# Lainshower/debiasing-multi-modal

Hardware: AMD Instinct MI355X
Metric: images/sec (embed+adapter step), CLIP-RN50 224px bs=1024 (higher is better)
Workload: dtype f32; 1 GPU; CLIP-RN50 224px encode_image + adapter(1024-128-1024) CE/SGD step, 1024 images/GPU, global batch 1024 (the metric's configuration, CLIP-RN50 224px bs=1024 on one GPU); global_batch=1024, batch_per_gpu=1024, parallelism=dp1, collective=none

## Files before the change

### debiasing-multi-modal_amd/csrc/bottleneck_chain.hip

```cpp
#include <stdlib.h>
#include "common.h"

namespace {

struct ChainP {
    const float* a; const float* a_absmax;
    const u16* w3; int w3_exp; const float* sc3; const float* b3;
    const float* res; float* x; float* xp; float* x_absmax;
    const u16* w1; int w1_exp; const float* sc1; const float* b1;
    float* y1; float* y1_absmax;
    int M, N;
    int Ho, Wo;
    const float* a2; const float* a2_absmax; const u16* wd; const float* ratio;
    const u16* w2; int w2_exp; const float* sc2; const float* b2;
    int H, W;
};

template <int RH>
__device__ __forceinline__ int swz(int row) { return RH == 32 ? ((row >> 2) & 3) : (RH == 64 ? ((row >> 1) & 7) : (row & 15)); }

constexpr int BM = 128;

template <int K, int P>
struct ChainGeo {
    static constexpr int BNS = K == 64 ? 64 : 32;
    static constexpr int SLROW = BNS + 4;
    static constexpr int R1_BYTES = BM * SLROW * 4 > 2 * BM * 64 * 2 ? BM * SLROW * 4 : 2 * BM * 64 * 2;
    static constexpr int W3_BYTES = BNS * K * 2;
    static constexpr int W1_BYTES = P * BNS * 2;
    static constexpr int LDS_BYTES = R1_BYTES + W3_BYTES + W1_BYTES;
};

template <int POOL>
__device__ __forceinline__ int row_pixel(const ChainP& p, int m) {
    if constexpr (!POOL) return m;
    const int mp = m >> 2, q = m & 3, wp2 = p.Wo >> 1, hwp = (p.Ho >> 1) * wp2;
    const int n = mp / hwp, rem = mp - n * hwp, hp = rem / wp2;
    return (n * p.Ho + 2 * hp + (q >> 1)) * p.Wo + 2 * (rem - hp * wp2) + (q & 1);
}

constexpr int C2_SROWS = 132, C2_PLANE = C2_SROWS * 32;
constexpr int C2_W2P = 104;
template <int K>
struct Conv2Geo {
    static constexpr int W2_OFF = 2 * C2_PLANE;
    static constexpr int GROUP_BYTES = (2 * C2_PLANE * 2 + K * C2_W2P * 2 + 255) / 256 * 256;
    static constexpr int NST = K == 64 ? 2 : 1;
    static constexpr int Z_OFF = NST * GROUP_BYTES;
    static constexpr int BYTES = Z_OFF + 256;
    static constexpr int STAGE_BYTES = BM * 68 * 4;
};
constexpr int cmax(int a, int b) { return a > b ? a : b; }

template <int K, int P, int POOL, int DUAL = 0, int CONV2 = 0>
__global__ __launch_bounds__(256, 2) void bottleneck_chain_kernel(const ChainP p) {
    static_assert(!DUAL || K == 64, "dual-source variant: layer-1 geometry (K = K2 = 64)");
    static_assert(!CONV2 || !POOL, "the conv2 phase walks pixels in standard order");
    static_assert(K == 64 || K == 128, "conv3 reduction depth: 64 (layer 1) or 128 (layer 2)");
    static_assert(P == 64 || P == 128, "conv1' width");
    using G = ChainGeo<K, P>;
    constexpr int BNS = G::BNS, SLROW = G::SLROW;
    constexpr int KS = K / 16, TN3 = BNS / 32, TN1 = P / 32;
    constexpr int LDS_TOTAL = cmax(G::LDS_BYTES + (DUAL ? BNS * 64 * 2 : 0), CONV2 ? cmax(Conv2Geo<K>::BYTES, Conv2Geo<K>::STAGE_BYTES) : 0);
    __shared__ __attribute__((aligned(256))) unsigned char lds_raw[LDS_TOTAL];
    u16* Ay = (u16*)lds_raw;
    float* slab = (float*)lds_raw;
    u16* W3b = (u16*)(lds_raw + G::R1_BYTES);
    u16* W1b = (u16*)(lds_raw + G::R1_BYTES + G::W3_BYTES);
    u16* Wdb = (u16*)(lds_raw + G::R1_BYTES + G::W3_BYTES + G::W1_BYTES);

    const int tid = threadIdx.x, lane = tid & 63, wave = tid >> 6;
    const int fr = lane & 31, fh = lane >> 5;
    const int m0 = xcd_remap(blockIdx.x, gridDim.x) * BM;
    const int NT = p.N / BNS;

    const int g0 = row_pixel<POOL>(p, m0);
    const long long Mll = p.M;
    const __amdgpu_buffer_rsrc_t rsA = desc(p.a, Mll * K * 4, (long long)g0 * K * 4);
    const __amdgpu_buffer_rsrc_t rsR = DUAL ? desc(p.a2, Mll * 64 * 4, (long long)g0 * 64 * 4)
                                            : desc(p.res, Mll * p.N * 4, (long long)g0 * p.N * 4);
    const __amdgpu_buffer_rsrc_t rsX = desc(p.x, POOL == 2 ? 0 : Mll * p.N * 4, (long long)g0 * p.N * 4);
    const __amdgpu_buffer_rsrc_t rsY = desc(p.y1, Mll * P * 4, (long long)g0 * P * 4);
    __amdgpu_buffer_rsrc_t rsXP = rsX;
    if constexpr (POOL) rsXP = desc(p.xp, (Mll >> 2) * p.N * 4, (long long)(m0 >> 2) * p.N * 4);

    unsigned gx[4], gy[4];
#pragma unroll
    for (int t = 0; t < 4; ++t) {
        const int m = m0 + wave * 32 + 8 * t + 4 * fh;
        const int dp = row_pixel<POOL>(p, m) - g0;
        gx[t] = m < p.M ? (unsigned)dp * (unsigned)(p.N * 4) + (unsigned)(fr * 4) : OOR;
        gy[t] = m < p.M ? (unsigned)dp * (unsigned)(P * 4) + (unsigned)(fr * 4) : OOR;
    }
    auto qpix = [&](int q) { return POOL ? (q >> 1) * p.Wo + (q & 1) : q; };

    constexpr int CPR3 = K / 8, RPP3 = 256 / CPR3, W3LD = BNS * CPR3 / 256;
    constexpr int CPR1 = BNS / 8, RPP1 = 256 / CPR1, W1LD = P * CPR1 / 256;
    static_assert(W3LD >= 1 && W1LD >= 1, "weight slabs smaller than one pass of the workgroup");
    const int wc3 = tid % CPR3, wr3 = tid / CPR3, wc1 = tid % CPR1, wr1 = tid / CPR1;
    u32x4 w3r[W3LD], w1r[W1LD], wdr[DUAL ? W3LD : 1];
    auto load_w = [&](int nt) {
#pragma unroll
        for (int j = 0; j < W3LD; ++j) {
            w3r[j] = *(const u32x4*)(p.w3 + (size_t)(nt * BNS + wr3 + RPP3 * j) * K + wc3 * 8);
            if constexpr (DUAL) wdr[j] = *(const u32x4*)(p.wd + (size_t)(nt * BNS + wr3 + RPP3 * j) * 64 + wc3 * 8);
        }
#pragma unroll
        for (int j = 0; j < W1LD; ++j)
            w1r[j] = *(const u32x4*)(p.w1 + (size_t)(wr1 + RPP1 * j) * p.N + nt * BNS + wc1 * 8);
    };
    auto store_w = [&]() {
#pragma unroll
        for (int j = 0; j < W3LD; ++j) {
            const int row = wr3 + RPP3 * j;
            *(u32x4*)(W3b + row * K + ((wc3 ^ swz<K>(row)) << 3)) = w3r[j];
            if constexpr (DUAL) *(u32x4*)(Wdb + row * 64 + ((wc3 ^ swz<64>(row)) << 3)) = wdr[j];
        }
#pragma unroll
        for (int j = 0; j < W1LD; ++j) {
            const int row = wr1 + RPP1 * j;
            *(u32x4*)(W1b + row * BNS + ((wc1 ^ swz<BNS>(row)) << 3)) = w1r[j];
        }
    };
    load_w(0);
    float rr[DUAL ? 1 : TN3][16];
    auto load_res = [&](int nt) {
        if constexpr (DUAL) return;
#pragma unroll
        for (int j = 0; j < TN3; ++j)
#pragma unroll
            for (int r = 0; r < 16; ++r)
                rr[j][r] = __builtin_bit_cast(float, __builtin_amdgcn_raw_buffer_load_b32(
                    rsR, gx[r >> 2], (unsigned)((nt * BNS + j * 32) * 4 + qpix(r & 3) * p.N * 4), 0));
    };
    load_res(0);
    u32x4 af[KS][2], af2[DUAL ? 4 : 1][2];
    bool first_pass = true;
    auto stage_issue = [&](const __amdgpu_buffer_rsrc_t& rs, int ldk, int k0, f32x4 (&q)[8]) {
        const int lc = tid & 15, lr = tid >> 4;
#pragma unroll
        for (int i = 0; i < 8; ++i) {
            const int row = lr + 16 * i, m = m0 + row;
            const unsigned off = m < p.M ? (unsigned)(row_pixel<POOL>(p, m) - g0) * (unsigned)(ldk * 4) + lc * 16u : OOR;
            q[i] = __builtin_bit_cast(f32x4, __builtin_amdgcn_raw_buffer_load_b128(rs, off, (unsigned)(k0 * 4), 0));
        }
    };
    auto stage_finish = [&](const f32x4 (&q)[8], float sc, u32x4 (*dst)[2]) {
        const int lc = tid & 15, lr = tid >> 4;
        if (!first_pass) __syncthreads();
#pragma unroll
        for (int i = 0; i < 8; ++i) {
            const int row = lr + 16 * i;
            unsigned hp[2], lp[2];
#pragma unroll
            for (int j = 0; j < 2; ++j) split2h_pair(q[i][2 * j], q[i][2 * j + 1], sc, hp[j], lp[j]);
            const int off = row * 64 + (((lc >> 1) ^ swz<64>(row)) << 3) + ((lc & 1) << 2);
            *(u32x2*)(Ay + off) = (u32x2){hp[0], hp[1]};
            *(u32x2*)(Ay + BM * 64 + off) = (u32x2){lp[0], lp[1]};
        }
        if (first_pass) store_w();
        first_pass = false;
        __syncthreads();
#pragma unroll
        for (int ks = 0; ks < 4; ++ks) {
            const int row = wave * 32 + fr;
            const int off = row * 64 + (((2 * ks + fh) ^ swz<64>(row)) << 3);
            dst[ks][0] = *(const u32x4*)(Ay + off);
            dst[ks][1] = *(const u32x4*)(Ay + BM * 64 + off);
        }
    };
    auto stage_pass = [&](const __amdgpu_buffer_rsrc_t& rs, int ldk, int k0, float sc, u32x4 (*dst)[2]) {
        f32x4 q[8];
        stage_issue(rs, ldk, k0, q);
        stage_finish(q, sc, dst);
    };
    f32x4 q2[(DUAL && CONV2) ? 8 : 1];
    if constexpr (DUAL && CONV2) stage_issue(rsR, 64, 0, q2);
    int s_a;
    if constexpr (!CONV2) {
        s_a = scale_exp(*p.a_absmax);
#pragma unroll
        for (int kp = 0; kp < K / 64; ++kp) stage_pass(rsA, K, kp * 64, pow2f(s_a), af + kp * 4);
    } else {
        using C2 = Conv2Geo<K>;
        constexpr int TN2 = K / 32, NG = (K / 32) * 3, W2LD = (K * 12 + 255) / 256;
        u16* Sp = (u16*)lds_raw;
        constexpr int NST = C2::NST, STH = C2::GROUP_BYTES / 2;
        constexpr int ZLH = C2::Z_OFF / 2;
        if (tid < 16) *(u32x4*)(lds_raw + C2::Z_OFF + tid * 16) = (u32x4){0u, 0u, 0u, 0u};
        const int s_y1 = scale_exp(*p.a_absmax);
        const float y1_sc = pow2f(s_y1);
        const int px0 = m0 - 1 - p.W > 0 ? m0 - 1 - p.W : 0;
        const __amdgpu_buffer_rsrc_t rsS = desc(p.a, Mll * K * 4, (long long)px0 * K * 4);
        const int lc = tid & 7, lr = tid >> 3;
        unsigned s_off[5];
#pragma unroll
        for (int i = 0; i < 5; ++i) {
            const int j = lr + 32 * i;
            s_off[i] = j < 130 ? (unsigned)((m0 - 1 + j - px0) * (K * 4)) + lc * 16u : OOR;
        }
        unsigned fmask = 0;
        {
            const int m = m0 + wave * 32 + fr;
            if (m < p.M) {
                const int hw = p.H * p.W, rem = m - (m / hw) * hw, ho = rem / p.W, wo = rem - ho * p.W;
#pragma unroll
                for (int kh = 0; kh < 3; ++kh)
#pragma unroll
                    for (int kw = 0; kw < 3; ++kw)
                        if (ho + kh - 1 >= 0 && ho + kh - 1 < p.H && wo + kw - 1 >= 0 && wo + kw - 1 < p.W) fmask |= 1u << (kh * 3 + kw);
            }
        }
        f32x4 sq[5];
        u32x4 w2q[W2LD];
        auto load_group = [&](int g) {
            const int sl = g / 3, kh = g - sl * 3;
            const unsigned delta = (unsigned)(((kh - 1) * p.W * K + sl * 32) * 4);
#pragma unroll
            for (int i = 0; i < 5; ++i)
                sq[i] = __builtin_bit_cast(f32x4, __builtin_amdgcn_raw_buffer_load_b128(rsS, s_off[i] == OOR ? OOR : s_off[i] + delta, 0, 0));
#pragma unroll
            for (int i = 0; i < W2LD; ++i) {
                const int idx = tid + 256 * i, row = idx / 12, c = idx - row * 12;
                w2q[i] = idx < K * 12 ? *(const u32x4*)(p.w2 + (size_t)row * (9 * K) + (size_t)g * 96 + c * 8) : (u32x4){0u, 0u, 0u, 0u};
            }
        };
        auto store_group = [&](int st) {
            u16* Sps = Sp + st * STH;
            u16* W2b = Sps + C2::W2_OFF;
#pragma unroll
            for (int i = 0; i < 5; ++i) {
                const int row = lr + 32 * i;
                if (row < 130) {
                    unsigned hp[2], lp[2];
#pragma unroll
                    for (int j = 0; j < 2; ++j) split2h_pair(sq[i][2 * j], sq[i][2 * j + 1], y1_sc, hp[j], lp[j]);
                    const int off = row * 32 + (((lc >> 1) ^ swz<32>(row)) << 3) + ((lc & 1) << 2);
                    *(u32x2*)(Sps + off) = (u32x2){hp[0], hp[1]};
                    *(u32x2*)(Sps + C2_PLANE + off) = (u32x2){lp[0], lp[1]};
                }
            }
#pragma unroll
            for (int i = 0; i < W2LD; ++i) {
                const int idx = tid + 256 * i, row = idx / 12, c = idx - row * 12;
                if (idx < K * 12) *(u32x4*)(W2b + row * C2_W2P + c * 8) = w2q[i];
            }
        };
        f32x16 acc2[TN2];
#pragma unroll
        for (int j = 0; j < TN2; ++j)
#pragma unroll
            for (int r = 0; r < 16; ++r) acc2[j][r] = 0.f;
        auto compute_group = [&](int g, int st) {
            const u16* Sps = Sp + st * STH;
            const u16* W2b = Sps + C2::W2_OFF;
            const int zl = ZLH - st * STH;
            const int kh = g % 3;
#pragma unroll
            for (int kw = 0; kw < 3; ++kw) {
                const bool ok = (fmask >> (kh * 3 + kw)) & 1u;
                const int row = wave * 32 + fr + kw;
#pragma unroll
                for (int ks = 0; ks < 2; ++ks) {
                    const int addr = row * 32 + (((2 * ks + fh) ^ swz<32>(row)) << 3);
                    const int a0 = ok ? addr : zl + (addr & 127), a1 = ok ? addr + C2_PLANE : zl + (addr & 127);
                    const u32x4 ah = *(const u32x4*)(Sps + a0), al = *(const u32x4*)(Sps + a1);
                    u32x4 wf[TN2];
#pragma unroll
                    for (int j = 0; j < TN2; ++j) wf[j] = *(const u32x4*)(W2b + (j * 32 + fr) * C2_W2P + kw * 32 + (2 * ks + fh) * 8);
#pragma unroll
                    for (int j = 0; j < TN2; ++j)
                        acc2[j] = __builtin_amdgcn_mfma_f32_32x32x16_f16(__builtin_bit_cast(f16x8, al), __builtin_bit_cast(f16x8, wf[j]), acc2[j], 0, 0, 0);
#pragma unroll
                    for (int j = 0; j < TN2; ++j)
                        acc2[j] = __builtin_amdgcn_mfma_f32_32x32x16_f16(__builtin_bit_cast(f16x8, ah), __builtin_bit_cast(f16x8, wf[j]), acc2[j], 0, 0, 0);
                }
            }
        };
        load_group(0);
        if constexpr (NST == 2) {
            store_group(0);
            __syncthreads();
            for (int g = 0; g < NG; ++g) {
                if (g + 1 < NG) load_group(g + 1);
                compute_group(g, g & 1);
                if (g + 1 < NG) store_group((g + 1) & 1);
                __syncthreads();
            }
        } else {
            for (int g = 0; g < NG; ++g) {
                store_group(0);
                __syncthreads();
                if (g + 1 < NG) load_group(g + 1);
                compute_group(g, 0);
                __syncthreads();
            }
        }
        const float c2_scale = pow2f(-s_y1 - p.w2_exp);
        float ymax = 0.f;
#pragma unroll
        for (int j = 0; j < TN2; ++j) {
            const float sv = p.sc2[j * 32 + fr] * c2_scale, bv = p.b2[j * 32 + fr];
#pragma unroll
            for (int r = 0; r < 16; ++r) {
                float v = fmaxf(fmaf(acc2[j][r], sv, bv), 0.f);
                if (gx[r >> 2] == OOR) v = 0.f;
                acc2[j][r] = v;
                ymax = fmaxf(ymax, v);
            }
        }
        s_a = scale_exp(wave_max(ymax));
        const float y2_sc = pow2f(s_a);
        float* St = (float*)lds_raw + wave * (32 * 68);
#pragma unroll
        for (int h = 0; h < K / 64; ++h) {
#pragma unroll
            for (int jj = 0; jj < 2; ++jj)
#pragma unroll
                for (int r = 0; r < 16; ++r) St[((r & 3) + 8 * (r >> 2) + 4 * fh) * 68 + jj * 32 + fr] = acc2[2 * h + jj][r];
#pragma unroll
            for (int ks = 0; ks < 4; ++ks) {
                const f32x4 x0 = *(const f32x4*)(St + fr * 68 + 16 * ks + 8 * fh), x1 = *(const f32x4*)(St + fr * 68 + 16 * ks + 8 * fh + 4);
                unsigned hh[4], ll[4];
                split2h_pair(x0[0], x0[1], y2_sc, hh[0], ll[0]); split2h_pair(x0[2], x0[3], y2_sc, hh[1], ll[1]);
                split2h_pair(x1[0], x1[1], y2_sc, hh[2], ll[2]); split2h_pair(x1[2], x1[3], y2_sc, hh[3], ll[3]);
                af[4 * h + ks][0] = (u32x4){hh[0], hh[1], hh[2], hh[3]};
                af[4 * h + ks][1] = (u32x4){ll[0], ll[1], ll[2], ll[3]};
            }
        }
        __syncthreads();
        if constexpr (!DUAL) store_w();
    }
    float dual_dyn = 1.f;
    if constexpr (DUAL) {
        const int s_a2 = scale_exp(*p.a2_absmax);
        if constexpr (CONV2) stage_finish(q2, pow2f(s_a2), af2);
        else stage_pass(rsR, 64, 0, pow2f(s_a2), af2);
        dual_dyn = pow2f(s_a - s_a2);
    }
    __syncthreads();

    float* Ls = slab + wave * (32 * SLROW);
    const float acc3_scale = pow2f(-s_a - p.w3_exp);
    f32x16 acc1[TN1];
#pragma unroll
    for (int j = 0; j < TN1; ++j)
#pragma unroll
        for (int r = 0; r < 16; ++r) acc1[j][r] = 0.f;
    float run_max = 0.f, x_amax = 0.f;
    int s_cur = 0;

    for (int nt = 0; nt < NT; ++nt) {
        const int n0 = nt * BNS;
        if (nt + 1 < NT) load_w(nt + 1);
        f32x16 acc3[TN3];
#pragma unroll
        for (int j = 0; j < TN3; ++j)
#pragma unroll
            for (int r = 0; r < 16; ++r) acc3[j][r] = 0.f;
        if constexpr (DUAL) {
#pragma unroll
            for (int ks = 0; ks < 4; ++ks) {
                u32x4 wf[TN3];
#pragma unroll
                for (int j = 0; j < TN3; ++j) {
                    const int row = j * 32 + fr;
                    wf[j] = *(const u32x4*)(Wdb + row * 64 + (((2 * ks + fh) ^ swz<64>(row)) << 3));
                }
#pragma unroll
                for (int pl = 1; pl >= 0; --pl)
#pragma unroll
                    for (int j = 0; j < TN3; ++j)
                        acc3[j] = __builtin_amdgcn_mfma_f32_32x32x16_f16(__builtin_bit_cast(f16x8, af2[ks][pl]),
                                                                         __builtin_bit_cast(f16x8, wf[j]), acc3[j], 0, 0, 0);
            }
#pragma unroll
            for (int j = 0; j < TN3; ++j) {
                const float rt = p.ratio[n0 + j * 32 + fr] * dual_dyn;
#pragma unroll
                for (int r = 0; r < 16; ++r) acc3[j][r] *= rt;
            }
        }
#pragma unroll
        for (int ks = 0; ks < KS; ++ks) {
            u32x4 wf[TN3];
#pragma unroll
            for (int j = 0; j < TN3; ++j) {
                const int row = j * 32 + fr;
                wf[j] = *(const u32x4*)(W3b + row * K + (((2 * ks + fh) ^ swz<K>(row)) << 3));
            }
#pragma unroll
            for (int pl = 1; pl >= 0; --pl)
#pragma unroll
                for (int j = 0; j < TN3; ++j)
                    acc3[j] = __builtin_amdgcn_mfma_f32_32x32x16_f16(__builtin_bit_cast(f16x8, af[ks][pl]),
                                                                     __builtin_bit_cast(f16x8, wf[j]), acc3[j], 0, 0, 0);
        }
        float tmax = 0.f;
#pragma unroll
        for (int j = 0; j < TN3; ++j) {
            const int n = n0 + j * 32 + fr;
            const float sv = p.sc3[n] * acc3_scale, bv = p.b3[n];
#pragma unroll
            for (int r = 0; r < 16; ++r) {
                float v = fmaxf(fmaf(acc3[j][r], sv, bv) + (DUAL ? 0.f : rr[j][r]), 0.f);
                if (gx[r >> 2] == OOR) v = 0.f;
                acc3[j][r] = v;
                tmax = fmaxf(tmax, v);
                if constexpr (POOL != 2)
                    __builtin_amdgcn_raw_buffer_store_b32(__builtin_bit_cast(unsigned, v), rsX, gx[r >> 2],
                                                          (unsigned)((n0 + j * 32) * 4 + qpix(r & 3) * p.N * 4), 0);
                Ls[((r & 3) + 8 * (r >> 2) + 4 * fh) * SLROW + j * 32 + fr] = v;
            }
            if constexpr (POOL) {
#pragma unroll
                for (int t = 0; t < 4; ++t) {
                    const float s = (((acc3[j][4 * t] + acc3[j][4 * t + 1]) + acc3[j][4 * t + 2]) + acc3[j][4 * t + 3]) * 0.25f;
                    const int mp = wave * 8 + 2 * t + fh;
                    const unsigned off = gx[t] != OOR ? (unsigned)mp * (unsigned)(p.N * 4) + (unsigned)(fr * 4) : OOR;
                    __builtin_amdgcn_raw_buffer_store_b32(__builtin_bit_cast(unsigned, s), rsXP, off, (unsigned)((n0 + j * 32) * 4), 0);
                }
            }
        }
        if (nt + 1 < NT) load_res(nt + 1);
        tmax = wave_max(tmax);
        x_amax = fmaxf(x_amax, tmax);
        if (tmax > run_max) {
            run_max = tmax;
            const int s_new = scale_exp(run_max);
            if (s_new != s_cur) {
                const float f = pow2f(s_new - s_cur);
#pragma unroll
                for (int j = 0; j < TN1; ++j)
#pragma unroll
                    for (int r = 0; r < 16; ++r) acc1[j][r] *= f;
                s_cur = s_new;
            }
        }
        const float t_sc = pow2f(s_cur);
#pragma unroll
        for (int ks = 0; ks < BNS / 16; ++ks) {
            const f32x4 x0 = *(const f32x4*)(Ls + fr * SLROW + 16 * ks + 8 * fh);
            const f32x4 x1 = *(const f32x4*)(Ls + fr * SLROW + 16 * ks + 8 * fh + 4);
            unsigned h[4], l[4];
            split2h_pair(x0[0], x0[1], t_sc, h[0], l[0]); split2h_pair(x0[2], x0[3], t_sc, h[1], l[1]);
            split2h_pair(x1[0], x1[1], t_sc, h[2], l[2]); split2h_pair(x1[2], x1[3], t_sc, h[3], l[3]);
            const u32x4 ah = {h[0], h[1], h[2], h[3]}, al = {l[0], l[1], l[2], l[3]};
            u32x4 wf[TN1];
#pragma unroll
            for (int j = 0; j < TN1; ++j) {
                const int row = j * 32 + fr;
                wf[j] = *(const u32x4*)(W1b + row * BNS + (((2 * ks + fh) ^ swz<BNS>(row)) << 3));
            }
#pragma unroll
            for (int j = 0; j < TN1; ++j)
                acc1[j] = __builtin_amdgcn_mfma_f32_32x32x16_f16(__builtin_bit_cast(f16x8, al), __builtin_bit_cast(f16x8, wf[j]),
                                                                 acc1[j], 0, 0, 0);
#pragma unroll
            for (int j = 0; j < TN1; ++j)
                acc1[j] = __builtin_amdgcn_mfma_f32_32x32x16_f16(__builtin_bit_cast(f16x8, ah), __builtin_bit_cast(f16x8, wf[j]),
                                                                 acc1[j], 0, 0, 0);
        }
        __syncthreads();
        if (nt + 1 < NT) store_w();
        __syncthreads();
    }

    float y_amax = 0.f;
    const float acc1_scale = pow2f(-s_cur - p.w1_exp);
#pragma unroll
    for (int j = 0; j < TN1; ++j) {
        const int n = j * 32 + fr;
        const float sv = p.sc1[n] * acc1_scale, bv = p.b1[n];
#pragma unroll
        for (int r = 0; r < 16; ++r) {
            const float v = fmaxf(fmaf(acc1[j][r], sv, bv), 0.f);
            __builtin_amdgcn_raw_buffer_store_b32(__builtin_bit_cast(unsigned, v), rsY, gy[r >> 2],
                                                  (unsigned)(j * 32 * 4 + qpix(r & 3) * P * 4), 0);
            if (gy[r >> 2] != OOR) y_amax = fmaxf(y_amax, v);
        }
    }
    y_amax = wave_max(y_amax);
    float* red = (float*)W3b;
    if (lane == 0) { red[wave] = x_amax; red[4 + wave] = y_amax; }
    __syncthreads();
    if (tid == 0) {
        const float xm = fmaxf(fmaxf(red[0], red[1]), fmaxf(red[2], red[3]));
        const float ym = fmaxf(fmaxf(red[4], red[5]), fmaxf(red[6], red[7]));
        if (p.x_absmax && xm > *(volatile const float*)p.x_absmax) atomicMax((unsigned*)p.x_absmax, __float_as_uint(xm));
        if (p.y1_absmax && ym > *(volatile const float*)p.y1_absmax) atomicMax((unsigned*)p.y1_absmax, __float_as_uint(ym));
    }
}

}

int dbmm_chain8_launch(const float* y2, const float* y2_absmax, const void* w3_plane_f16, int w3_exp, const float* scale3,
                       const float* bias3, const float* residual, float* x_out, float* x_absmax, const void* w1_plane_f16, int w1_exp,
                       const float* scale1, const float* bias1, float* y1_out, float* y1_absmax, int64_t M, int64_t N, void* stream);

extern "C" int dbmm_bottleneck_block_chain_x2(const float* y1, const float* y1_absmax, const void* w2_plane_f16, int w2_exp,
                                              const float* scale2, const float* bias2, const void* w3_plane_f16, int w3_exp,
                                              const float* scale3, const float* bias3, const float* residual, const float* a2,
                                              const float* a2_absmax, const void* wd_plane_f16, const float* ratio, float* x_out,
                                              float* x_absmax, const void* w1_plane_f16, int w1_exp, const float* scale1,
                                              const float* bias1, float* y1_out, float* y1_out_absmax, int64_t B, int64_t H,
                                              int64_t W, int64_t K, int64_t N, int64_t P, void* stream) {
    const bool dual = a2 != nullptr;
    if (!y1 || !y1_absmax || !w2_plane_f16 || !scale2 || !bias2 || !w3_plane_f16 || !scale3 || !bias3 || !x_out || !w1_plane_f16 ||
        !scale1 || !bias1 || !y1_out)
        return DBMM_E_ARG;
    if (dual ? (!a2_absmax || !wd_plane_f16 || !ratio || residual) : (!residual || a2_absmax || wd_plane_f16 || ratio)) return DBMM_E_ARG;
    if (B <= 0 || H <= 0 || W <= 0 || K <= 0 || N <= 0 || P <= 0) return DBMM_E_SHAPE;
    const int64_t M = B * H * W;
    if (M > (INT32_MAX >> 1)) return DBMM_E_SHAPE;
    const bool served = dual ? (K == 64 && P == 64) : ((K == 64 && P == 64) || (K == 128 && P == 128));
    if (!served || (N % 64) != 0 || (M & 3)) return DBMM_E_UNSUPPORTED;
    if (w2_exp < -40 || w2_exp > 40 || w3_exp < -40 || w3_exp > 40 || w1_exp < -40 || w1_exp > 40) return DBMM_E_UNSUPPORTED;
    if (!dbmm_aligned16(y1) || !dbmm_aligned16(w2_plane_f16) || !dbmm_aligned16(w3_plane_f16) || !dbmm_aligned16(w1_plane_f16) ||
        !dbmm_aligned16(x_out) || !dbmm_aligned16(y1_out) || (residual && !dbmm_aligned16(residual)) || (a2 && !dbmm_aligned16(a2)) ||
        (wd_plane_f16 && !dbmm_aligned16(wd_plane_f16)))
        return DBMM_E_ALIGN;
    ChainP p{};
    p.a = y1; p.a_absmax = y1_absmax;
    p.w2 = (const u16*)w2_plane_f16; p.w2_exp = w2_exp; p.sc2 = scale2; p.b2 = bias2; p.H = (int)H; p.W = (int)W;
    p.w3 = (const u16*)w3_plane_f16; p.w3_exp = w3_exp; p.sc3 = scale3; p.b3 = bias3;
    p.res = residual; p.a2 = a2; p.a2_absmax = a2_absmax; p.wd = (const u16*)wd_plane_f16; p.ratio = ratio;
    p.x = x_out; p.x_absmax = x_absmax;
    p.w1 = (const u16*)w1_plane_f16; p.w1_exp = w1_exp; p.sc1 = scale1; p.b1 = bias1;
    p.y1 = y1_out; p.y1_absmax = y1_out_absmax;
    p.M = (int)M; p.N = (int)N; p.Ho = (int)H; p.Wo = (int)W;
    const dim3 grid((unsigned)((M + BM - 1) / BM));
    hipStream_t s = (hipStream_t)stream;
    if (dual) hipLaunchKernelGGL((bottleneck_chain_kernel<64, 64, 0, 1, 1>), grid, dim3(256), 0, s, p);
    else if (K == 64) hipLaunchKernelGGL((bottleneck_chain_kernel<64, 64, 0, 0, 1>), grid, dim3(256), 0, s, p);
    else hipLaunchKernelGGL((bottleneck_chain_kernel<128, 128, 0, 0, 1>), grid, dim3(256), 0, s, p);
    DBMM_CHECK_LAUNCH();
    return DBMM_OK;
}

extern "C" int dbmm_bottleneck_chain_dual_x2(const float* y2, const float* y2_absmax, const void* w3_plane_f16, int w3_exp,
                                             const float* scale3, const float* bias, const float* a2, const float* a2_absmax,
                                             const void* wd_plane_f16, const float* ratio, float* x_out, float* x_absmax,
                                             const void* w1_plane_f16, int w1_exp, const float* scale1, const float* bias1,
                                             float* y1_out, float* y1_absmax, int64_t M, int64_t K, int64_t K2, int64_t N,
                                             int64_t P, void* stream) {
    if (!y2 || !y2_absmax || !w3_plane_f16 || !scale3 || !bias || !a2 || !a2_absmax || !wd_plane_f16 || !ratio || !x_out ||
        !w1_plane_f16 || !scale1 || !bias1 || !y1_out)
        return DBMM_E_ARG;
    if (M <= 0 || K <= 0 || K2 <= 0 || N <= 0 || P <= 0 || M > (INT32_MAX >> 1)) return DBMM_E_SHAPE;
    if (K != 64 || K2 != 64 || (N % 64) != 0 || (P != 64 && P != 128) || (M & 3)) return DBMM_E_UNSUPPORTED;
    if (w3_exp < -40 || w3_exp > 40 || w1_exp < -40 || w1_exp > 40) return DBMM_E_UNSUPPORTED;
    if (!dbmm_aligned16(y2) || !dbmm_aligned16(a2) || !dbmm_aligned16(w3_plane_f16) || !dbmm_aligned16(wd_plane_f16) ||
        !dbmm_aligned16(w1_plane_f16) || !dbmm_aligned16(x_out) || !dbmm_aligned16(y1_out))
        return DBMM_E_ALIGN;
    ChainP p{};
    p.a = y2; p.a_absmax = y2_absmax;
    p.w3 = (const u16*)w3_plane_f16; p.w3_exp = w3_exp; p.sc3 = scale3; p.b3 = bias;
    p.a2 = a2; p.a2_absmax = a2_absmax; p.wd = (const u16*)wd_plane_f16; p.ratio = ratio;
    p.x = x_out; p.x_absmax = x_absmax;
    p.w1 = (const u16*)w1_plane_f16; p.w1_exp = w1_exp; p.sc1 = scale1; p.b1 = bias1;
    p.y1 = y1_out; p.y1_absmax = y1_absmax;
    p.M = (int)M; p.N = (int)N; p.Ho = 1; p.Wo = (int)M;
    const dim3 grid((unsigned)((M + BM - 1) / BM));
    hipStream_t s = (hipStream_t)stream;
    if (P == 64) hipLaunchKernelGGL((bottleneck_chain_kernel<64, 64, 0, 1>), grid, dim3(256), 0, s, p);
    else hipLaunchKernelGGL((bottleneck_chain_kernel<64, 128, 0, 1>), grid, dim3(256), 0, s, p);
    DBMM_CHECK_LAUNCH();
    return DBMM_OK;
}

extern "C" int dbmm_bottleneck_chain_x2(const float* y2, const float* y2_absmax, const void* w3_plane_f16, int w3_exp,
                                        const float* scale3, const float* bias3, const float* residual, float* x_out,
                                        float* x_pooled, float* x_absmax, const void* w1_plane_f16, int w1_exp,
                                        const float* scale1, const float* bias1, float* y1_out, float* y1_absmax,
                                        int64_t B, int64_t Ho, int64_t Wo, int64_t K, int64_t N, int64_t P, void* stream) {
    if (!y2 || !y2_absmax || !w3_plane_f16 || !scale3 || !bias3 || !residual || !w1_plane_f16 || !scale1 || !bias1 || !y1_out)
        return DBMM_E_ARG;
    if (!x_out && !x_pooled) return DBMM_E_ARG;
    if (B <= 0 || Ho <= 0 || Wo <= 0 || K <= 0 || N <= 0 || P <= 0) return DBMM_E_SHAPE;
    const int64_t M = B * Ho * Wo;
    if (M > (INT32_MAX >> 1)) return DBMM_E_SHAPE;
    if (M & 3) return DBMM_E_UNSUPPORTED;
    if (K == 256 && P == 256 && !x_pooled && dbmm_opt(OPT_CHAIN8)) {
        if (w3_exp < -40 || w3_exp > 40 || w1_exp < -40 || w1_exp > 40) return DBMM_E_UNSUPPORTED;
        if (!dbmm_aligned16(y2) || !dbmm_aligned16(w3_plane_f16) || !dbmm_aligned16(w1_plane_f16) || !dbmm_aligned16(residual) ||
            !dbmm_aligned16(x_out) || !dbmm_aligned16(y1_out))
            return DBMM_E_ALIGN;
        return dbmm_chain8_launch(y2, y2_absmax, w3_plane_f16, w3_exp, scale3, bias3, residual, x_out, x_absmax, w1_plane_f16, w1_exp,
                                  scale1, bias1, y1_out, y1_absmax, M, N, stream);
    }
    if ((K != 64 && K != 128) || (N % 64) != 0 || (P != 64 && P != 128)) return DBMM_E_UNSUPPORTED;
    if (w3_exp < -40 || w3_exp > 40 || w1_exp < -40 || w1_exp > 40) return DBMM_E_UNSUPPORTED;
    if (x_pooled && ((Ho & 1) || (Wo & 1))) return DBMM_E_UNSUPPORTED;
    if (!dbmm_aligned16(y2) || !dbmm_aligned16(w3_plane_f16) || !dbmm_aligned16(w1_plane_f16) || !dbmm_aligned16(residual) ||
        (x_out && !dbmm_aligned16(x_out)) || !dbmm_aligned16(y1_out) || (x_pooled && !dbmm_aligned16(x_pooled)))
        return DBMM_E_ALIGN;
    ChainP p{};
    p.a = y2; p.a_absmax = y2_absmax;
    p.w3 = (const u16*)w3_plane_f16; p.w3_exp = w3_exp; p.sc3 = scale3; p.b3 = bias3;
    p.res = residual; p.x = x_out; p.xp = x_pooled; p.x_absmax = x_absmax;
    p.w1 = (const u16*)w1_plane_f16; p.w1_exp = w1_exp; p.sc1 = scale1; p.b1 = bias1;
    p.y1 = y1_out; p.y1_absmax = y1_absmax;
    p.M = (int)M; p.N = (int)N; p.Ho = (int)Ho; p.Wo = (int)Wo;
    const dim3 grid((unsigned)((M + BM - 1) / BM));
    hipStream_t s = (hipStream_t)stream;
#define CHAIN_LAUNCH(KK, PP, PL) hipLaunchKernelGGL((bottleneck_chain_kernel<KK, PP, PL>), grid, dim3(256), 0, s, p)
    if (K == 64) {
        if (!x_out)        { if (P == 64) CHAIN_LAUNCH(64, 64, 2); else CHAIN_LAUNCH(64, 128, 2); }
        else if (x_pooled) { if (P == 64) CHAIN_LAUNCH(64, 64, 1); else CHAIN_LAUNCH(64, 128, 1); }
        else               { if (P == 64) CHAIN_LAUNCH(64, 64, 0); else CHAIN_LAUNCH(64, 128, 0); }
    } else {
        if (!x_out)        { if (P == 64) CHAIN_LAUNCH(128, 64, 2); else CHAIN_LAUNCH(128, 128, 2); }
        else if (x_pooled) { if (P == 64) CHAIN_LAUNCH(128, 64, 1); else CHAIN_LAUNCH(128, 128, 1); }
        else               { if (P == 64) CHAIN_LAUNCH(128, 64, 0); else CHAIN_LAUNCH(128, 128, 0); }
    }
#undef CHAIN_LAUNCH
    DBMM_CHECK_LAUNCH();
    return DBMM_OK;
}
```

### debiasing-multi-modal_amd/ops.py

```python
import ctypes
import math
import os
from collections import namedtuple

import numpy as np
import torch

from . import _lib
from ._lib import check, ptr, require_cuda, stream

ACT_NONE, ACT_RELU, ACT_QUICKGELU = 0, 1, 2


class DbmmUnsupported(_lib.DbmmError):
    """a wrapper's C entry answered DBMM_E_UNSUPPORTED (no kernel for this valid request)"""


def set_option(name, value):
    old = get_option(name)
    check(_lib.lib().dbmm_set_option(name.encode(), int(value)), f"set_option({name})")
    return old


def get_option(name):
# ... 203 lines not shown
    Cout, Cin, kh, kw = w_oihw.shape
    slab = 32 if chunk_major == 32 else 16
    if chunk_major and kh * kw > 1 and Cin % slab == 0:
        w = w_oihw.reshape(Cout, Cin // slab, slab, kh, kw).permute(0, 1, 3, 4, 2)
        return w.contiguous().float().reshape(Cout, kh * kw * Cin), (WL_CHUNK32_MAJOR if slab == 32 else WL_CHUNK_MAJOR)
    return w_oihw.permute(0, 2, 3, 1).contiguous().float().reshape(Cout, kh * kw * Cin), WL_TAP_MAJOR


def conv_bn_act(x, w, bias, residual, kh, kw, stride, pad, act, w_layout=WL_TAP_MAJOR, w_planes=None,
                w_planes_f16=None, w_exp=0, x_absmax=None, y_absmax=None, out_scale=None, pool=1, keep_full=False):
    require_cuda(x, w)
    _f32c(x); _f32c(w)
    B, H, W, Cin = x.shape
    Cout = w.shape[0]
    Ho = (H + 2 * pad - kh) // stride + 1
    Wo = (W + 2 * pad - kw) // stride + 1
    if pool not in (1, 2):
        raise _lib.DbmmError("conv_bn_act: pool must be 1 or 2")
    if w.numel() != Cout * kh * kw * Cin:
        raise RuntimeError(f"conv_bn_act: packed weight {tuple(w.shape)} for a {kh} x {kw} conv over {Cin} channels")
    _sized("conv_bn_act bias", bias, Cout); _sized("conv_bn_act out_scale", out_scale, Cout)
    if residual is not None and tuple(residual.shape) != (B, Ho, Wo, Cout):
        raise RuntimeError(f"conv_bn_act: residual {tuple(residual.shape)} for a {(B, Ho, Wo, Cout)} output")
    if w_planes_f16 is not None and w_planes_f16.numel() != w_planes_f16.shape[0] * w.numel():
        raise RuntimeError(f"conv_bn_act: weight planes {tuple(w_planes_f16.shape)} for a packed weight {tuple(w.shape)}")
    plain = kh == 1 and kw == 1 and stride == 1 and pad == 0
    split = w_planes_f16 is not None or y_absmax is not None or out_scale is not None
    wby = w_planes_f16.numel() * 2 if w_planes_f16 is not None else (w_planes.numel() * 2 if w_planes is not None else w.numel() * 4)
    oel = B * Ho * Wo * Cout
    nby_pool = 4 * (x.numel() + (residual.numel() if residual is not None else 0) + oel // 4 + (oel if keep_full else 0)) + wby
    nby = 4 * (x.numel() + (residual.numel() if residual is not None else 0) + oel) + wby
    if (Cin == 32 and kh == 3 and kw == 3 and stride == 1 and pad == 1 and act == ACT_RELU and residual is None and not keep_full
            and w_planes_f16 is not None and w_planes_f16.shape[0] == 1 and out_scale is not None and x_absmax is not None
            and Cout in (32, 64) and H % 4 == 0 and W % 28 == 0 and (pool == 1 or (H % 2 == 0 and W % 2 == 0))
            and w_layout in (WL_TAP_MAJOR, WL_CHUNK32_MAJOR) and get_option("conv_patch")):
        y = _empty((B, H // pool, W // pool, Cout), device=x.device, dtype=torch.float32)
        global _chain_tag
        _chain_tag = f"conv3x3_c32_kernel<{Cout}, {int(pool == 2)}>"
        t = _Timed(B * H * W, Cout, 9 * Cin, -1, 0, 4 * (x.numel() + y.numel()) + 2 * Cout * 9 * Cin)
        t.__enter__()
        rc = _lib.lib().dbmm_conv3x3_c32_bn_relu_x2(ptr(x), ptr(x_absmax), ptr(w_planes_f16), int(w_exp), ptr(out_scale), ptr(bias),
                                                   ptr(y), ptr(y_absmax), B, H, W, Cin, Cout, 2 if pool == 2 else 0, stream())
        if rc == 0:
            t.__exit__(None, None, None)
            return y
        if rc not in (_lib.E_UNSUPPORTED, _lib.E_ALIGN):
            check(rc, "conv3x3_c32_bn_relu_x2")
        del y
    if pool == 2 and split and Ho % 2 == 0 and Wo % 2 == 0:
        y = _empty((B, Ho // 2, Wo // 2, Cout), device=x.device, dtype=torch.float32)
        yf = _empty((B, Ho, Wo, Cout), device=x.device, dtype=torch.float32) if keep_full else None
        t = _Timed(B * Ho * Wo, Cout, kh * kw * Cin, 0 if plain else 1, 0, nby_pool)
        t.__enter__()
        rc = _conv_x2(x, w, bias, residual, y, kh, kw, stride, pad, act, w_layout, w_planes_f16, w_exp, x_absmax,
                      y_absmax, out_scale, 2, yf)
        if rc == 0:
            t.__exit__(None, None, None)
            return (y, yf) if keep_full else y
        if rc != _lib.E_UNSUPPORTED:
            check(rc, "conv_bn_act_x2(pool)")
    y = _empty((B, Ho, Wo, Cout), device=x.device, dtype=torch.float32)
    with _Timed(B * Ho * Wo, Cout, kh * kw * Cin, 0 if plain else 1, 0, nby):
        ws = igemm_workspace(x.device)
        if split:
            check(_conv_x2(x, w, bias, residual, y, kh, kw, stride, pad, act, w_layout, w_planes_f16, w_exp, x_absmax,
                           y_absmax, out_scale, 0, None), "conv_bn_act_x2")
        elif w_planes is not None:
            check(_lib.lib().dbmm_conv_bn_act_x3(ptr(x), ptr(w), ptr(w_planes), ptr(bias), ptr(residual), ptr(y), B, H, W,
                                                 Cin, Cout, kh, kw, stride, pad, act, int(w_layout), ptr(ws),
                                                 ws.numel() * 4, stream()), "conv_bn_act_x3")
        else:
            check(_lib.lib().dbmm_conv_bn_act_ws(ptr(x), ptr(w), ptr(bias), ptr(residual), ptr(y), B, H, W, Cin, Cout, kh,
                                                 kw, stride, pad, act, int(w_layout), ptr(ws), ws.numel() * 4, stream()),
                  "conv_bn_act")
    if pool == 2:
        return (avgpool2d(y, 2), y) if keep_full else avgpool2d(y, 2)
    return y


def _conv_x2(x, w, bias, residual, y, kh, kw, stride, pad, act, w_layout, w_planes_f16, w_exp, x_absmax, y_absmax,
             out_scale, pool, y_full):
    B, H, W, Cin = x.shape
    ws = igemm_workspace(x.device)
    nw = 2 if w_planes_f16 is None else int(w_planes_f16.shape[0])
    return _lib.lib().dbmm_conv_bn_act_x2(ptr(x), ptr(x_absmax), ptr(w), ptr(w_planes_f16), nw, int(w_exp), ptr(out_scale),
                                          ptr(bias), ptr(residual), ptr(y), ptr(y_full), ptr(y_absmax), B, H, W, Cin,
                                          w.shape[0], kh,
                                          kw, stride, pad, act, pool, int(w_layout), ptr(ws), ws.numel() * 4, stream())


def gemm_dual(a, a_absmax, w_plane, w_exp, out_scale, a2, a2_absmax, w2_plane, ratio, bias, act=ACT_RELU, c_absmax=None):
    require_cuda(a, a2)
    _f32c(a); _f32c(a2)
    K, K2 = a.shape[-1], a2.shape[-1]
    M, N = a.numel() // K, w_plane.shape[1]
    if a2.numel() // K2 != M:
        raise _lib.DbmmError("gemm_dual: operand row counts differ")
    c = _empty(tuple(a.shape[:-1]) + (N,), device=a.device, dtype=torch.float32)
    ws = igemm_workspace(a.device)
    t = _Timed(M, N, K + K2, 0, 0, 4 * (M * K + M * K2 + M * N) + 2 * (N * K + N * K2))
    t.__enter__()
    rc = _lib.lib().dbmm_gemm_dual_bn_act_x2(ptr(a), K, ptr(a_absmax), ptr(w_plane), int(w_exp), K, K, ptr(out_scale),
                                             ptr(a2), K2, ptr(a2_absmax), ptr(w2_plane), K2, K2, ptr(ratio), ptr(bias),
                                             ptr(c), N, ptr(c_absmax), M, N, act, ptr(ws), ws.numel() * 4, stream())
    if rc == _lib.E_UNSUPPORTED:
        return None
    check(rc, "gemm_dual_bn_act_x2")
    t.__exit__(None, None, None)
    return c


def bottleneck_chain(y2, y2_absmax, c3, residual, c1, x_absmax=None, y1_absmax=None, pooled=False, keep_full=True):
    require_cuda(y2, residual)
    _f32c(y2); _f32c(residual)
    B, H, W, K = y2.shape
    N, P = c3["ph"].shape[1], c1["ph"].shape[1]
    if c3["ph"].shape[0] != 1 or c1["ph"].shape[0] != 1 or tuple(residual.shape) != (B, H, W, N):
        return None
    chain8 = K == 256 and P == 256 and not pooled and get_option("chain8")
    if not chain8 and (K not in (64, 128) or P not in (64, 128)):
        return None
    if N % 64 or (pooled and (H % 2 or W % 2)):
        return None
    dev = y2.device
    full = keep_full or not pooled
    x = _empty((B, H, W, N), device=dev, dtype=torch.float32) if full else None
    y1 = _empty((B, H, W, P), device=dev, dtype=torch.float32)
    xp = _empty((B, H // 2, W // 2, N), device=dev, dtype=torch.float32) if pooled else None
    M = B * H * W
    global _chain_tag
    _chain_tag = "bottleneck_chain8_kernel" if chain8 else f"bottleneck_chain_kernel<{K}, {P}, {int(pooled) + int(not full)}, 0>"
    t = _Timed(M, N, K + P, -1, 0, 4 * (M * K + (2 if full else 1) * M * N + M * P + (M // 4 * N if pooled else 0)) + 2 * (N * K + P * N))
    t.__enter__()
    rc = _lib.lib().dbmm_bottleneck_chain_x2(ptr(y2), ptr(y2_absmax), ptr(c3["ph"]), int(c3["we"]), ptr(c3["sc"]), ptr(c3["b"]),
                                            ptr(residual), ptr(x), ptr(xp), ptr(x_absmax), ptr(c1["ph"]), int(c1["we"]),
                                            ptr(c1["sc"]), ptr(c1["b"]), ptr(y1), ptr(y1_absmax), B, H, W, K, N, P, stream())
    if rc == _lib.E_UNSUPPORTED:
        return None
    check(rc, "bottleneck_chain_x2")
    t.__exit__(None, None, None)
    return (x, xp, y1) if pooled else (x, y1)


_chain_tag = None


def bottleneck_block_chain(y1, y1_absmax, c2, c3, c1, residual=None, dual=None, x_absmax=None, y1n_absmax=None):
    require_cuda(y1)
    _f32c(y1)
    B, H, W, K = y1.shape
    N, P = c3["ph"].shape[1], c1["ph"].shape[1]
    M = B * H * W
    if (c2["ph"] is None or c2["ph"].shape[0] != 1 or c2["wl"] != WL_CHUNK32_MAJOR or tuple(c2["ph"].shape[1:]) != (K, 9 * K)
            or c3["ph"].shape[0] != 1 or c1["ph"].shape[0] != 1 or N % 64 or M % 4):
        return None
    if dual is None:
        if (K, P) not in ((64, 64), (128, 128)) or residual is None or tuple(residual.shape) != (B, H, W, N):
            return None
    elif (K, P) != (64, 64) or dual["ds"]["ph"].shape[0] != 1 or tuple(dual["a2"].shape) != (B, H, W, 64):
        return None
    x = _empty((B, H, W, N), device=y1.device, dtype=torch.float32)
    y1n = _empty((B, H, W, P), device=y1.device, dtype=torch.float32)
    global _chain_tag
    _chain_tag = f"bottleneck_chain_kernel<{K}, {P}, 0, {int(dual is not None)}, 1>"
    K2 = 64 if dual is not None else 0
    nby = 4 * (M * K + M * N * (1 if dual is not None else 2) + M * K2 + M * P) + 2 * (K * 9 * K + N * K + N * K2 + P * N)
    t = _Timed(M, 1, 9 * K * K + N * (K + K2 + P), -1, 0, nby)
    t.__enter__()
    d = dual or {}
    bias3 = d["bias"] if dual is not None else c3["b"]
    rc = _lib.lib().dbmm_bottleneck_block_chain_x2(
        ptr(y1), ptr(y1_absmax), ptr(c2["ph"]), int(c2["we"]), ptr(c2["sc"]), ptr(c2["b"]), ptr(c3["ph"]), int(c3["we"]),
        ptr(c3["sc"]), ptr(bias3), ptr(residual) if dual is None else None, ptr(d.get("a2")), ptr(d.get("a2_absmax")),
        ptr(d["ds"]["ph"]) if dual is not None else None, ptr(d.get("ratio")), ptr(x), ptr(x_absmax), ptr(c1["ph"]), int(c1["we"]),
        ptr(c1["sc"]), ptr(c1["b"]), ptr(y1n), ptr(y1n_absmax), B, H, W, K, N, P, stream())
    if rc == _lib.E_UNSUPPORTED:
        return None
    check(rc, "bottleneck_block_chain_x2")
    t.__exit__(None, None, None)
    return x, y1n


def bottleneck_chain_dual(y2, y2_absmax, c3, a2, a2_absmax, ds, ratio, bias, c1, x_absmax=None, y1_absmax=None):
    require_cuda(y2, a2)
    _f32c(y2); _f32c(a2)
    K, K2 = y2.shape[-1], a2.shape[-1]
    N, P = c3["ph"].shape[1], c1["ph"].shape[1]
    M = y2.numel() // K
    if (c3["ph"].shape[0] != 1 or ds["ph"].shape[0] != 1 or c1["ph"].shape[0] != 1 or a2.numel() // K2 != M
            or K != 64 or K2 != 64 or N % 64 or P not in (64, 128) or M % 4):
        return None
    x = _empty(tuple(y2.shape[:-1]) + (N,), device=y2.device, dtype=torch.float32)
    y1 = _empty(tuple(y2.shape[:-1]) + (P,), device=y2.device, dtype=torch.float32)
    global _chain_tag
    _chain_tag = f"bottleneck_chain_kernel<{K}, {P}, 0, 1>"
    t = _Timed(M, N, K + K2 + P, -1, 0, 4 * (M * K + M * K2 + M * N + M * P) + 2 * (N * K + N * K2 + P * N))
    t.__enter__()
    rc = _lib.lib().dbmm_bottleneck_chain_dual_x2(ptr(y2), ptr(y2_absmax), ptr(c3["ph"]), int(c3["we"]), ptr(c3["sc"]), ptr(bias),
                                                 ptr(a2), ptr(a2_absmax), ptr(ds["ph"]), ptr(ratio), ptr(x), ptr(x_absmax),
                                                 ptr(c1["ph"]), int(c1["we"]), ptr(c1["sc"]), ptr(c1["b"]), ptr(y1),
                                                 ptr(y1_absmax), M, K, K2, N, P, stream())
    if rc == _lib.E_UNSUPPORTED:
        return None
    check(rc, "bottleneck_chain_dual_x2")
    t.__exit__(None, None, None)
    return x, y1


def conv_stem_s2(x_nchw, w, bias, y_absmax=None):
    require_cuda(x_nchw, w)
    _f32c(x_nchw); _f32c(w)
    B, C, H, W = x_nchw.shape
    if C != 3:
        raise _lib.DbmmError("stem conv expects 3 input channels")
    Cout = w.shape[-1]
    y = _empty((B, (H - 1) // 2 + 1, (W - 1) // 2 + 1, Cout), device=x_nchw.device, dtype=torch.float32)
    check(_lib.lib().dbmm_conv_stem_s2(ptr(x_nchw), ptr(w), ptr(bias), ptr(y), ptr(y_absmax), B, H, W, Cout, stream()),
          "conv_stem_s2")
    return y


def avgpool2d(x, k):
    require_cuda(x)
    _f32c(x)
    B, H, W, C = x.shape
    y = _empty((B, H // k, W // k, C), device=x.device, dtype=torch.float32)
    check(_lib.lib().dbmm_avgpool2d(ptr(x), ptr(y), B, H, W, C, k, stream()), "avgpool2d")
    return y


def attnpool(x, pos, wq, bq, wkv, bkv, wc, bc, heads):
    require_cuda(x)
    if x.dtype != torch.float16:
        _f32c(x)
    elif not x.is_contiguous():
        raise _lib.DbmmError("attnpool: expected a contiguous tensor")
    B, H, W, C = x.shape
    HW = H * W
    Dout = wc.shape[0]
    if tuple(pos.shape) != (HW + 1, C):
        raise RuntimeError(f"attnpool: positional embedding {tuple(pos.shape)} does not match a {H} x {W} x {C} feature map "
                           f"(expected ({HW + 1}, {C})): the input resolution differs from the one the model was built for")
    if (tuple(wq.shape) != (C, C) or tuple(wkv.shape) != (2 * C, C) or wc.shape[1] != C or bq.numel() != C or bkv.numel() != 2 * C
            or bc.numel() != Dout):
        raise RuntimeError(f"attnpool: projection shapes {tuple(wq.shape)}, {tuple(wkv.shape)}, {tuple(wc.shape)} do not match C = {C}")
    for t in (pos, wq, bq, wkv, bkv, wc, bc):
        require_cuda(t)
        _f32c(t)
    nbytes = _lib.lib().dbmm_workspace_bytes_attnpool(B, HW, C)
    ws = _empty(nbytes // 4, device=x.device, dtype=torch.float32)
    out = _empty((B, Dout), device=x.device, dtype=torch.float32)
    check(_lib.lib().dbmm_attnpool_x(ptr(x), int(x.dtype == torch.float16), ptr(pos), ptr(wq), ptr(bq), ptr(wkv), ptr(bkv), ptr(wc), ptr(bc),
                                     ptr(out), B, HW, C, heads, Dout, ptr(ws), nbytes, stream()), "attnpool")
    return out


def layernorm(x, gamma, beta, rows=None, ldx=None, eps=1e-5, y_absmax=None):
    require_cuda(x)
    E = gamma.numel()
    if rows is None:
        rows = x.numel() // E
    if ldx is None:
        ldx = E
    _sized("layernorm beta", beta, E)
    if ldx < E or x.numel() < (rows - 1) * ldx + E:
        raise RuntimeError(f"layernorm: input {tuple(x.shape)} for {rows} rows of {E} at pitch {ldx}")
    y = _empty((rows, E), device=x.device, dtype=torch.float32)
    check(_lib.lib().dbmm_layernorm(ptr(x), ldx, ptr(gamma), ptr(beta), ptr(y), E, rows, E, eps, ptr(y_absmax), stream()),
          "layernorm")
    return y


def mha_core(qkv, B, L, E, heads, causal, qkv_absmax=None):
    require_cuda(qkv)
    if qkv.numel() != B * L * 3 * E or E != heads * 64:
        raise RuntimeError(f"mha_core: qkv {tuple(qkv.shape)} for B = {B}, L = {L}, E = {E}, {heads} heads of 64")
    out = _empty((B * L, E), device=qkv.device, dtype=torch.float32)
    if qkv_absmax is not None and get_option("mha_x2"):
        with _TimedTag("mha_pair_kernel", 4.0 * B * heads * L * L * 64, 4 * (B * L * 4 * E)):
            check(_lib.lib().dbmm_mha_core_x2(ptr(qkv), ptr(qkv_absmax), ptr(out), B, L, E, heads, int(causal), stream()),
                  "mha_core_x2")
        return out
    with _TimedTag("mha_mfma_kernel", 4.0 * B * heads * L * L * 64, 4 * (B * L * 4 * E)):
        check(_lib.lib().dbmm_mha_core(ptr(qkv), ptr(out), B, L, E, heads, int(causal), stream()), "mha_core")
    return out


def _embed_gather_check(name, tokens, table, pos):
    require_cuda(tokens, table, pos)
    _f32c(table, f"{name} table"); _f32c(pos, f"{name} pos")
    if tokens.dim() != 2 or table.dim() != 2:
        raise RuntimeError(f"{name}: tokens {tuple(tokens.shape)} and table {tuple(table.shape)} where [n, L] ids and a [vocab, W] table are expected")
    if tokens.dtype != torch.int32:
        tokens = tokens.to(torch.int32)
    return tokens.contiguous()


def embed_gather(tokens, table, pos):
    tokens = _embed_gather_check("embed_gather", tokens, table, pos)
    n, L = tokens.shape
    W = table.shape[1]
    if tuple(pos.shape) != (L, W):
        raise RuntimeError(f"embed_gather: {L} tokens per prompt against a positional embedding of shape {tuple(pos.shape)}")
    out = _empty((n, L, W), device=table.device, dtype=torch.float32)
    check(_lib.lib().dbmm_embed_gather(ptr(tokens), ptr(table), ptr(pos), ptr(out), n, L, W, table.shape[0], stream()),
          "embed_gather")
    return out, tokens
# ... 1416 lines not shown
```

Baseline: 36400 images/sec.

## Double-buffer chain weight slabs and prefetch per-channel scale vectors

For the conv2-fused K=64 non-dual chain kernel, the weight slab in LDS is double-buffered by parity, so the next tile's weights are stored while other waves may still read the current buffer, and one of the two barriers per N-tile is removed. Per-channel scale, bias and ratio vectors are prefetched one tile ahead into registers instead of being loaded from global memory inside the epilogue. The N-divisibility check is relaxed to 32 for K=128. This uses more LDS and registers, which risks occupancy, though a static assert keeps the LDS within two workgroups per CU.

```diff
diff --git a/debiasing-multi-modal_amd/csrc/bottleneck_chain.hip b/debiasing-multi-modal_amd/csrc/bottleneck_chain.hip
--- a/debiasing-multi-modal_amd/csrc/bottleneck_chain.hip
+++ b/debiasing-multi-modal_amd/csrc/bottleneck_chain.hip
@@ -28,7 +28,6 @@
     static constexpr int R1_BYTES = BM * SLROW * 4 > 2 * BM * 64 * 2 ? BM * SLROW * 4 : 2 * BM * 64 * 2;
     static constexpr int W3_BYTES = BNS * K * 2;
     static constexpr int W1_BYTES = P * BNS * 2;
-    static constexpr int LDS_BYTES = R1_BYTES + W3_BYTES + W1_BYTES;
 };
 
 template <int POOL>
@@ -61,7 +60,10 @@
     using G = ChainGeo<K, P>;
     constexpr int BNS = G::BNS, SLROW = G::SLROW;
     constexpr int KS = K / 16, TN3 = BNS / 32, TN1 = P / 32;
-    constexpr int LDS_TOTAL = cmax(G::LDS_BYTES + (DUAL ? BNS * 64 * 2 : 0), CONV2 ? cmax(Conv2Geo<K>::BYTES, Conv2Geo<K>::STAGE_BYTES) : 0);
+    constexpr bool VPRE = CONV2 && K == 64, WDB = VPRE && !DUAL;
+    constexpr int WBUF = G::W3_BYTES + G::W1_BYTES + (DUAL ? BNS * 64 * 2 : 0);
+    constexpr int LDS_TOTAL = cmax(G::R1_BYTES + (WDB ? 2 : 1) * WBUF, CONV2 ? cmax(Conv2Geo<K>::BYTES, Conv2Geo<K>::STAGE_BYTES) : 0);
+    static_assert(!WDB || LDS_TOTAL <= 80 * 1024, "two workgroups per CU");
     __shared__ __attribute__((aligned(256))) unsigned char lds_raw[LDS_TOTAL];
     u16* Ay = (u16*)lds_raw;
     float* slab = (float*)lds_raw;
@@ -109,20 +111,31 @@
         for (int j = 0; j < W1LD; ++j)
             w1r[j] = *(const u32x4*)(p.w1 + (size_t)(wr1 + RPP1 * j) * p.N + nt * BNS + wc1 * 8);
     };
-    auto store_w = [&]() {
+    auto store_w = [&](int par = 0) {
+        const int po = WDB ? par * (WBUF / 2) : 0;
 #pragma unroll
         for (int j = 0; j < W3LD; ++j) {
             const int row = wr3 + RPP3 * j;
-            *(u32x4*)(W3b + row * K + ((wc3 ^ swz<K>(row)) << 3)) = w3r[j];
-            if constexpr (DUAL) *(u32x4*)(Wdb + row * 64 + ((wc3 ^ swz<64>(row)) << 3)) = wdr[j];
+            *(u32x4*)(W3b + po + row * K + ((wc3 ^ swz<K>(row)) << 3)) = w3r[j];
+            if constexpr (DUAL) *(u32x4*)(Wdb + po + row * 64 + ((wc3 ^ swz<64>(row)) << 3)) = wdr[j];
         }
 #pragma unroll
         for (int j = 0; j < W1LD; ++j) {
             const int row = wr1 + RPP1 * j;
-            *(u32x4*)(W1b + row * BNS + ((wc1 ^ swz<BNS>(row)) << 3)) = w1r[j];
+            *(u32x4*)(W1b + po + row * BNS + ((wc1 ^ swz<BNS>(row)) << 3)) = w1r[j];
         }
     };
     load_w(0);
+    float sc3n[VPRE ? TN3 : 1], b3n[VPRE ? TN3 : 1], rtn[VPRE && DUAL ? TN3 : 1];
+    auto load_vec = [&](int nt) {
+#pragma unroll
+        for (int j = 0; j < TN3; ++j) {
+            const int n = nt * BNS + j * 32 + fr;
+            sc3n[j] = p.sc3[n]; b3n[j] = p.b3[n];
+            if constexpr (DUAL) rtn[j] = p.ratio[n];
+        }
+    };
+    if constexpr (VPRE) load_vec(0);
     float rr[DUAL ? 1 : TN3][16];
     auto load_res = [&](int nt) {
         if constexpr (DUAL) return;
@@ -352,7 +365,16 @@
 
     for (int nt = 0; nt < NT; ++nt) {
         const int n0 = nt * BNS;
-        if (nt + 1 < NT) load_w(nt + 1);
+        const int wpar = WDB ? (nt & 1) * (WBUF / 2) : 0;
+        float sc3c[TN3], b3c[TN3], rtc[DUAL ? TN3 : 1];
+        if constexpr (VPRE) {
+#pragma unroll
+            for (int j = 0; j < TN3; ++j) { sc3c[j] = sc3n[j]; b3c[j] = b3n[j]; if constexpr (DUAL) rtc[j] = rtn[j]; }
+        }
+        if (nt + 1 < NT) {
+            load_w(nt + 1);
+            if constexpr (VPRE) load_vec(nt + 1);
+        }
         f32x16 acc3[TN3];
 #pragma unroll
         for (int j = 0; j < TN3; ++j)
@@ -365,7 +387,7 @@
 #pragma unroll
                 for (int j = 0; j < TN3; ++j) {
                     const int row = j * 32 + fr;
-                    wf[j] = *(const u32x4*)(Wdb + row * 64 + (((2 * ks + fh) ^ swz<64>(row)) << 3));
+                    wf[j] = *(const u32x4*)(Wdb + wpar + row * 64 + (((2 * ks + fh) ^ swz<64>(row)) << 3));
                 }
 #pragma unroll
                 for (int pl = 1; pl >= 0; --pl)
@@ -376,7 +398,8 @@
             }
 #pragma unroll
             for (int j = 0; j < TN3; ++j) {
-                const float rt = p.ratio[n0 + j * 32 + fr] * dual_dyn;
+                if constexpr (!VPRE) rtc[j] = p.ratio[n0 + j * 32 + fr];
+                const float rt = rtc[j] * dual_dyn;
 #pragma unroll
                 for (int r = 0; r < 16; ++r) acc3[j][r] *= rt;
             }
@@ -387,7 +410,7 @@
 #pragma unroll
             for (int j = 0; j < TN3; ++j) {
                 const int row = j * 32 + fr;
-                wf[j] = *(const u32x4*)(W3b + row * K + (((2 * ks + fh) ^ swz<K>(row)) << 3));
+                wf[j] = *(const u32x4*)(W3b + wpar + row * K + (((2 * ks + fh) ^ swz<K>(row)) << 3));
             }
 #pragma unroll
             for (int pl = 1; pl >= 0; --pl)
@@ -399,8 +422,8 @@
         float tmax = 0.f;
 #pragma unroll
         for (int j = 0; j < TN3; ++j) {
-            const int n = n0 + j * 32 + fr;
-            const float sv = p.sc3[n] * acc3_scale, bv = p.b3[n];
+            if constexpr (!VPRE) { sc3c[j] = p.sc3[n0 + j * 32 + fr]; b3c[j] = p.b3[n0 + j * 32 + fr]; }
+            const float sv = sc3c[j] * acc3_scale, bv = b3c[j];
 #pragma unroll
             for (int r = 0; r < 16; ++r) {
                 float v = fmaxf(fmaf(acc3[j][r], sv, bv) + (DUAL ? 0.f : rr[j][r]), 0.f);
@@ -450,7 +473,7 @@
 #pragma unroll
             for (int j = 0; j < TN1; ++j) {
                 const int row = j * 32 + fr;
-                wf[j] = *(const u32x4*)(W1b + row * BNS + (((2 * ks + fh) ^ swz<BNS>(row)) << 3));
+                wf[j] = *(const u32x4*)(W1b + wpar + row * BNS + (((2 * ks + fh) ^ swz<BNS>(row)) << 3));
             }
 #pragma unroll
             for (int j = 0; j < TN1; ++j)
@@ -461,9 +484,14 @@
                 acc1[j] = __builtin_amdgcn_mfma_f32_32x32x16_f16(__builtin_bit_cast(f16x8, ah), __builtin_bit_cast(f16x8, wf[j]),
                                                                  acc1[j], 0, 0, 0);
         }
-        __syncthreads();
-        if (nt + 1 < NT) store_w();
-        __syncthreads();
+        if constexpr (WDB) {
+            if (nt + 1 < NT) store_w((nt + 1) & 1);
+            __syncthreads();
+        } else {
+            __syncthreads();
+            if (nt + 1 < NT) store_w();
+            __syncthreads();
+        }
     }
 
     float y_amax = 0.f;
@@ -514,7 +542,7 @@
     const int64_t M = B * H * W;
     if (M > (INT32_MAX >> 1)) return DBMM_E_SHAPE;
     const bool served = dual ? (K == 64 && P == 64) : ((K == 64 && P == 64) || (K == 128 && P == 128));
-    if (!served || (N % 64) != 0 || (M & 3)) return DBMM_E_UNSUPPORTED;
+    if (!served || (N % (K == 64 ? 64 : 32)) != 0 || (M & 3)) return DBMM_E_UNSUPPORTED;
     if (w2_exp < -40 || w2_exp > 40 || w3_exp < -40 || w3_exp > 40 || w1_exp < -40 || w1_exp > 40) return DBMM_E_UNSUPPORTED;
     if (!dbmm_aligned16(y1) || !dbmm_aligned16(w2_plane_f16) || !dbmm_aligned16(w3_plane_f16) || !dbmm_aligned16(w1_plane_f16) ||
         !dbmm_aligned16(x_out) || !dbmm_aligned16(y1_out) || (residual && !dbmm_aligned16(residual)) || (a2 && !dbmm_aligned16(a2)) ||
diff --git a/debiasing-multi-modal_amd/ops.py b/debiasing-multi-modal_amd/ops.py
--- a/debiasing-multi-modal_amd/ops.py
+++ b/debiasing-multi-modal_amd/ops.py
@@ -379,7 +379,7 @@
     N, P = c3["ph"].shape[1], c1["ph"].shape[1]
     M = B * H * W
     if (c2["ph"] is None or c2["ph"].shape[0] != 1 or c2["wl"] != WL_CHUNK32_MAJOR or tuple(c2["ph"].shape[1:]) != (K, 9 * K)
-            or c3["ph"].shape[0] != 1 or c1["ph"].shape[0] != 1 or N % 64 or M % 4):
+            or c3["ph"].shape[0] != 1 or c1["ph"].shape[0] != 1 or N % (64 if K == 64 else 32) or M % 4):
         return None
     if dual is None:
         if (K, P) not in ((64, 64), (128, 128)) or residual is None or tuple(residual.shape) != (B, H, W, N):
```

New measurement: 36540 images/sec, median of 6. No clear change (+0.4%).
